# matthieugomez/LeastSquaresOptim.jl

Hardware: AMD Instinct MI355X
Metric: lm_lsmr_outer_iterations_per_sec (higher is better)
Workload: dtype f64

## Files before the change

### leastsquaresoptim.jl_amd/csrc/lsq_optimize.hip

```cpp
#include <chrono>
#include <cmath>
#include <cstring>

#include "lsq_solver.h"
#include "lsq_spmv.h"

static constexpr double MIN_DELTA = 1e-16, MAX_DELTA = 1e16, MIN_STEP_QUALITY = 1e-3;
static constexpr double MIN_DIAGONAL = 1e-6, MAX_DIAGONAL = 1e32;
static constexpr double DECREASE_THRESHOLD = 0.25, INCREASE_THRESHOLD = 0.75;

enum { SL_GRAD = 8, SL_DX = 9, SL_NONFIN = 10, SL_TRIAL = 11, SL_PRED = 12, SL_SSR = 13, SL_W0 = 14, SL_W1 = 15,
       SL_W2 = 16, SL_SUM = 17 };

extern "C" int lsq_solver_create(lsq_ctx *c, lsq_mat *J, int kind, int for_lm, lsq_solver **out) {
    LSQ_RANGE("lsq_solver_create");
    if (!c || !J || !out) return LSQ_EARG;
    if (kind == LSQ_QR && J->kind != LSQ_MAT_DENSE) {
        lsq_set_error("solver QR() is not available for sparse Jacobians. Choose between Cholesky() and LSMR()");
        return LSQ_EARG;
    }
    const bool blockdiag = kind == LSQ_CHOLESKY && J->kind == LSQ_MAT_CSC && J->bd_blocks > 0;
    const bool bordered = kind == LSQ_CHOLESKY && J->kind == LSQ_MAT_CSC && J->br_blocks > 0;
    if (kind == LSQ_CHOLESKY && J->kind != LSQ_MAT_DENSE && !blockdiag && !bordered) {
        lsq_set_error("MethodError: no AbstractAllocatedSolver for Cholesky() with a sparse Jacobian "
// ... 597 lines not shown
            (void)o->allreduce(v, 3, o->allreduce_user);
        }
        return st;
    }
};

#define CB(call)                                          \
    do {                                                  \
        if ((call) != 0) {                                \
            lsq_set_error("user callback reported failure"); \
            return LSQ_ECALLBACK;                         \
        }                                                 \
    } while (0)

static int call_g(lsq_g_callback g, lsq_mat *J, const double *x, void *user) {
    J->version++;
    if (J->kind == LSQ_MAT_CSC && !J->d_cs_user) J->csr_fresh = false;
    CB(g(J, x, user));
    return lsq_ensure_csr(J);
}
int lsq_call_g(lsq_g_callback g, lsq_mat *J, const double *x, void *user) { return call_g(g, J, x, user); }

struct IterateGuard {
    lsq_ctx *c;
    double *&x, *&fcur;
    double *x_user, *fcur_user;
    int m, n;
    ~IterateGuard() {
        if (x != x_user) lsq_d2d(c, x_user, x, (size_t)n * sizeof(double));
        if (fcur != fcur_user) lsq_d2d(c, fcur_user, fcur, (size_t)m * sizeof(double));
    }
};

static int start_residual(lsq_ctx *c, lsq_mat *J, lsq_f_callback f, void *user, double *fcur, const double *x, double *ssr,
                          int *nonfinite_at) {
    const int m = J->m, n = J->n;
    if (lsq_small_mat(J) || lsq_small_vec(m) || m <= 0) {
        CB(f(fcur, x, user));
        LSQ_TRY(lsq_sumsq(c, m, fcur, ssr));
        return lsq_first_nonfinite(c, n, x, nonfinite_at);
    }
    static_assert(SL_TRIAL == SL_NONFIN + 1, "the two scalars of the loop head travel together");
    LSQ_TRY(lsq_first_nonfinite_to_slot(c, n, x, c->d_slots + SL_NONFIN));
    LSQ_TRY(f_then_sumsq(c, false, f, user, m, fcur, x, 7, c->d_slots + SL_TRIAL));
    double sl[2];
    LSQ_TRY(lsq_read_slots(c, SL_NONFIN, 2, sl));
    *nonfinite_at = (int)sl[0];
    *ssr = sl[1];
    return LSQ_OK;
}

static int optimize_lm_loop(lsq_ctx *c, lsq_solver *sv, LoopBuffers &b, lsq_mat *J, double *x_user, double *fcur_user,
                            lsq_f_callback f, lsq_g_callback g, void *user, const lsq_options *o, lsq_result *r);
static int optimize_lm(lsq_ctx *c, lsq_solver *sv, LoopBuffers &b, lsq_mat *J, double *x_user, double *fcur_user,
                       lsq_f_callback f, lsq_g_callback g, void *user, const lsq_options *o, lsq_result *r) {
    ShardedExit ex{c, o};
    return ex.finish(optimize_lm_loop(c, sv, b, J, x_user, fcur_user, f, g, user, o, r));
}
static int optimize_lm_loop(lsq_ctx *c, lsq_solver *sv, LoopBuffers &b, lsq_mat *J, double *x_user, double *fcur_user,
                            lsq_f_callback f, lsq_g_callback g, void *user, const lsq_options *o, lsq_result *r) {
    const int m = J->m, n = J->n;
    double *x = x_user, *fcur = fcur_user, *xt = b.xt, *ftrial = b.ftrial;
    IterateGuard guard{c, x, fcur, x_user, fcur_user, m, n};
    double delta = o->delta > 0 ? o->delta : 10.0;
    double decrease_factor = 2.0;
    int f_calls = 0, g_calls = 0, mul_calls = 0, xc = 0, fc = 0, gc = 0;
    bool converged = false;
    double ssr;
    int iter = 0, nonfinite_at = -1;
    const bool sharded = o->row_allreduce != nullptr;
    if (sharded) CB(f(fcur, x, user));
    else LSQ_TRY(start_residual(c, J, f, user, fcur, x, &ssr, &nonfinite_at));
    f_calls++;
    auto rows_sum = [&](double *d_buf, int count) -> int {
        if (o->row_allreduce(d_buf, count, (void *)c->stream, o->row_allreduce_user) != 0) {
            lsq_set_error("row all-reduce callback reported failure");
            return LSQ_ECALLBACK;
        }
        return LSQ_OK;
    };
    if (sharded) {
        LSQ_TRY(sumsq_to_slot(c, false, m, fcur, 7, c->d_slots + SL_TRIAL));
        LSQ_TRY(rows_sum(c->d_slots + SL_TRIAL, 1));
        LSQ_TRY(lsq_read_slots(c, SL_TRIAL, 1, &ssr));
        LSQ_TRY(lsq_first_nonfinite(c, n, x, &nonfinite_at));
    }
    r->ssr0 = ssr;
    double maxabs_gr = INFINITY;
    bool need_jac = true;
    const int gn = ngrid(c, n);
    const bool exact = lsq_small_mat(J) && !sharded && !(sv->kind == LSQ_LSMR && sv->gen_ldiv);
    int last_inner = 0;
    const bool no_spec_grad = getenv("LSQ_NO_SPEC_GRADIENT") != nullptr;
    bool spec_launched = false, spec_grad_ready = false, spec_pending = false;
    struct SpecGuard { lsq_mat *J; bool &ready; bool &pending; ~SpecGuard() { if (ready || pending) lsq_sparse_colsum_forget(J); } }
        spec_guard{J, spec_grad_ready, spec_pending};
    int local_done = 0;
    double gssr = ssr, ggr = maxabs_gr;
    long long inner_total = 0;
    while (iter < o->iterations) {
        if (!o->allreduce && converged) break;
        if (o->allreduce && converged) {
            int all = 1;
            gssr = ssr; ggr = maxabs_gr;
            LSQ_TRY(global_exchange(o, &gssr, &ggr, &all));
            if (all) break;
            ++iter; local_done = 1;
            continue;
        }
        iter++;
        if (nonfinite_at >= 0) {
            r->bad_index = nonfinite_at;
            r->iterations = iter - 1;
            lsq_set_error("IsFiniteException: non-finite x at index %d", nonfinite_at);
            return LSQ_ENONFINITE;
        }
        if (need_jac) {
            LSQ_TRY(call_g(g, J, x, user));
            g_calls++;
            need_jac = false;
        }
        bool have_grad = false;
        if (spec_grad_ready) {
            lsq_sparse_grad_colsum_adopt(J);
            have_grad = true;
            spec_grad_ready = false;
        }
        const bool spec_ok = !no_spec_grad && !exact && !sharded && sv->kind == LSQ_LSMR && f == model_f && g == model_g &&
                             iter < o->iterations && !lsq_dbg_serial;
        spec_launched = false;
        if (!exact && J->colsum_version != J->version && lsq_can_fuse_grad_colsum(J)) {
            LSQ_TRY(lsq_sparse_grad_colsum(J, fcur, b.grad));
            have_grad = true;
        }
        const double *cs = nullptr;
        LSQ_TRY(lsq_rowshard_colsum(sv, J, &cs));
        const bool one_wg = !exact && n <= LSQ_ONE_WG_N;
        const bool lm_prep = one_wg && sv->kind == LSQ_LSMR && ssr >= 0.0 && lsq_lsmr_takes_lm_prep(sv, J);
        if (exact) LSQ_TRY(lsq_exact_lm_damp(c, n, cs, 1.0 / delta, b.dtd));
        else if (!one_wg) LSQ_LAUNCH(k_lm_damp, dim3(1), dim3(1024), 0, c->stream, n, cs, 1.0 / delta, b.dtd);
        {
            if (!have_grad) LSQ_TRY(gradient_into(c, exact, J, fcur, b.grad));
            if (sharded) LSQ_TRY(rows_sum(b.grad, n));
            if (lm_prep) {}
            else if (one_wg)
                LSQ_LAUNCH(k_lm_damp_grad, dim3(1), dim3(1024), 0, c->stream, n, cs, 1.0 / delta, b.dtd, b.grad,
                                   x, b.lo, b.hi, c->d_slots + SL_GRAD);
            else
                LSQ_LAUNCH(k_gradnorm, dim3(gn), dim3(LSQ_NT), 0, c->stream, n, b.grad, x, b.lo, b.hi,
                                   c->d_partials, lsq_ctr(c, 4), c->d_slots + SL_GRAD);
            mul_calls++;
        }
        struct Xchg { const lsq_options *o; double *gssr, *ggr; } xchg{o, &gssr, &ggr};
        if (o->allreduce) {
            gssr = ssr; ggr = maxabs_gr;
            c->idle_hook = [](void *p) -> int {
                Xchg *q = (Xchg *)p;
                int all = 0;
                return global_exchange(q->o, q->gssr, q->ggr, &all);
            };
            c->idle_user = &xchg;
            c->idle_status = 0;
            if (sv->kind != LSQ_LSMR || exact) lsq_run_idle_hook(c);
        }
        int lmiter = 0;
        struct TailCtx {
// ... 108 lines not shown
            decrease_factor *= 2.0;
        }
        record(o, c, iter, n, ssr, maxabs_gr, delta, rho, lmiter, accepted ? 1 : 0, x);
    }
    (void)local_done;
    LSQ_HIP(hipStreamSynchronize(c->stream));
    r->optimizer = LSQ_LEVENBERG_MARQUARDT;
    r->ssr = o->allreduce ? gssr : ssr;
    r->iterations = iter;
    r->converged = converged; r->x_converged = xc; r->f_converged = fc; r->g_converged = gc;
    r->f_calls = f_calls; r->g_calls = g_calls; r->mul_calls = mul_calls;
    r->lsmr_iterations = inner_total;
    return LSQ_OK;
}

static int optimize_dogleg_loop(lsq_ctx *c, lsq_solver *sv, LoopBuffers &b, lsq_mat *J, double *x, double *fcur,
                                lsq_f_callback f, lsq_g_callback g, void *user, const lsq_options *o, lsq_result *r);
static int optimize_dogleg(lsq_ctx *c, lsq_solver *sv, LoopBuffers &b, lsq_mat *J, double *x, double *fcur,
                           lsq_f_callback f, lsq_g_callback g, void *user, const lsq_options *o, lsq_result *r) {
    ShardedExit ex{c, o};
    return ex.finish(optimize_dogleg_loop(c, sv, b, J, x, fcur, f, g, user, o, r));
}
static int optimize_dogleg_loop(lsq_ctx *c, lsq_solver *sv, LoopBuffers &b, lsq_mat *J, double *x_user, double *fcur_user,
                                lsq_f_callback f, lsq_g_callback g, void *user, const lsq_options *o, lsq_result *r) {
    const int m = J->m, n = J->n;
    double *x = x_user, *fcur = fcur_user, *xt = b.xt, *ftrial = b.ftrial;
    IterateGuard guard{c, x, fcur, x_user, fcur_user, m, n};
    double delta = o->delta > 0 ? o->delta : 1.0;
    bool reuse = false, converged = false;
    double wnorm_dgn = 0.0, wnorm_dgr = 0.0, alpha = 0.0, wdot_gr_gn = 0.0;
    int f_calls = 0, g_calls = 0, mul_calls = 0, xc = 0, fc = 0, gc = 0;
    double ssr;
    int iter = 0, nonfinite_at = -1;
    LSQ_TRY(start_residual(c, J, f, user, fcur, x, &ssr, &nonfinite_at));
    f_calls++;
    r->ssr0 = ssr;
    double maxabs_gr = INFINITY;
    const int gn = ngrid(c, n);
    const bool exact = lsq_small_mat(J);
    double gssr = ssr, ggr = maxabs_gr;
    long long inner_total = 0;
    while (iter < o->iterations) {
        if (!o->allreduce && converged) break;
        if (o->allreduce && converged) {
            int all = 1;
            gssr = ssr; ggr = maxabs_gr;
            LSQ_TRY(global_exchange(o, &gssr, &ggr, &all));
            if (all) break;
            ++iter;
            continue;
        }
        iter++;
        if (nonfinite_at >= 0) {
            r->bad_index = nonfinite_at;
            r->iterations = iter - 1;
            lsq_set_error("IsFiniteException: non-finite x at index %d", nonfinite_at);
            return LSQ_ENONFINITE;
        }
        int ls_iter = 0;
        bool exchanged = false;
        if (!reuse) {
            LSQ_TRY(call_g(g, J, x, user));
            g_calls++;
            bool have_grad = false;
            if (!exact && J->colsum_version != J->version && lsq_can_fuse_grad_colsum(J)) {
                LSQ_TRY(lsq_sparse_grad_colsum(J, fcur, b.dgr));
                have_grad = true;
            }
            const double *cs = lsq_cached_colsum(J);
            if (!cs) return LSQ_EHIP;
            LSQ_LAUNCH(k_dl_scale, dim3(gn), dim3(LSQ_NT), 0, c->stream, n, cs, b.dtd);
            if (iter == 1) {
                double wx2;
                LSQ_TRY(lsq_wdot(c, n, x, x, b.dtd, &wx2));
                double wx = std::sqrt(wx2);
                if (wx > 0) delta *= wx;
            }
            if (!have_grad) LSQ_TRY(gradient_into(c, exact, J, fcur, b.dgr));
            mul_calls++;
            LSQ_LAUNCH(k_gradnorm, dim3(gn), dim3(LSQ_NT), 0, c->stream, n, b.dgr, x, b.lo, b.hi,
                               c->d_partials, lsq_ctr(c, 4), c->d_slots + SL_GRAD);
            LSQ_TRY(lsq_ediv(c, n, b.dgr, b.dtd, b.dgr));
            LSQ_TRY(wdot_to_slot(c, exact, n, b.dgr, b.dgr, b.dtd, 5, c->d_slots + SL_W0));
            LSQ_TRY(predicted_to_slot(c, exact, J, b.dgr, nullptr, b.fpred, 6, c->d_slots + SL_SUM));
            mul_calls++;
            LSQ_TRY(lsq_fill(c, n, 0.0, b.dgn));
            if (o->allreduce) {
                int all = 0;
                gssr = ssr; ggr = maxabs_gr;
                LSQ_TRY(global_exchange(o, &gssr, &ggr, &all));
                exchanged = true;
            }
            if (sv->kind == LSQ_LSMR) LSQ_TRY(lsq_lsmr_solve(sv, J, fcur, nullptr, b.dgn, &ls_iter));
            else LSQ_TRY(lsq_ldiv(sv, J, fcur, b.dgn, &ls_iter));
            mul_calls += ls_iter;
            inner_total += ls_iter / 2;
            LSQ_TRY(wdot_to_slot(c, exact, n, b.dgn, b.dgn, b.dtd, 5, c->d_slots + SL_W1));
            LSQ_TRY(wdot_to_slot(c, exact, n, b.dgr, b.dgn, b.dtd, 5, c->d_slots + SL_W2));
            LSQ_HIP(hipGetLastError());
            double sl10[10];
// ... 92 lines not shown
        LSQ_TRY(lsq_d2h(c, hx.data(), x, (size_t)n * sizeof(double)));
        int st = check_start(hx.data(), n, opt);
        if (st != LSQ_OK) {
            lsq_set_error("ArgumentError: Initial guess must be within bounds.");
            res->status = st;
            return st;
        }
    }
    LsqWorkspace *w = (LsqWorkspace *)c->workspace;
    const bool lm = optimizer == LSQ_LEVENBERG_MARQUARDT;
    if (!(w && w->J == J && w->m == J->m && w->n == J->n && w->optimizer == optimizer && w->solver_kind == solver_kind &&
          w->has_lo == (opt->h_lower != nullptr) && w->has_hi == (opt->h_upper != nullptr))) {
        lsq_workspace_free(w);
        c->workspace = nullptr;
        w = new LsqWorkspace();
        int st0 = lsq_solver_create(c, J, solver_kind, lm, &w->solver);
        if (st0 != LSQ_OK) {
            delete w;
            res->status = st0;
            return st0;
        }
        w->buf = new LoopBuffers();
        st0 = alloc_loop(*w->buf, c, J->m, J->n, opt, !lm);
        if (st0 != LSQ_OK) {
            lsq_workspace_free(w);
            res->status = st0;
            return st0;
        }
        w->J = J; w->m = J->m; w->n = J->n; w->optimizer = optimizer; w->solver_kind = solver_kind;
        w->has_lo = opt->h_lower != nullptr; w->has_hi = opt->h_upper != nullptr;
        c->workspace = w;
    } else {
        const size_t nb = (size_t)(J->n > 0 ? J->n : 1) * sizeof(double);
        LSQ_HIP(hipMemsetAsync(w->buf->dx, 0, nb, c->stream));
        if (opt->h_lower) LSQ_HIP(hipMemcpyAsync(w->buf->lo, opt->h_lower, nb, hipMemcpyHostToDevice, c->stream));
        if (opt->h_upper) LSQ_HIP(hipMemcpyAsync(w->buf->hi, opt->h_upper, nb, hipMemcpyHostToDevice, c->stream));
        if (opt->h_lower || opt->h_upper) LSQ_HIP(hipStreamSynchronize(c->stream));
    }
    if (w->solver->kind == LSQ_LSMR) {
        w->solver->precond_cb = opt->preconditioner;
        w->solver->precond_user = opt->preconditioner_user;
        w->solver->gen_update = opt->precond_update;
        w->solver->gen_ldiv = opt->precond_ldiv;
        w->solver->gen_user = opt->precond_general_user;
    }
    if (opt->row_allreduce) {
        if (!lm || w->solver->kind != LSQ_LSMR || opt->allreduce || J->kind == LSQ_MAT_OP) {
            lsq_set_error("row-sharded runs (lsq_options.row_allreduce): LevenbergMarquardt(LSMR()) on stored Jacobians only, and "
                          "not together with the independent-problems exchange (lsq_options.allreduce)");
            res->status = LSQ_EARG;
            return LSQ_EARG;
        }
        LSQ_TRY(lsq_solver_set_row_allreduce(w->solver, opt->row_allreduce, opt->row_allreduce_user,
                                             opt->global_rows > 0 ? opt->global_rows : (long long)J->m));
    } else if (w->solver->kind == LSQ_LSMR) {
        LSQ_TRY(lsq_solver_set_row_allreduce(w->solver, nullptr, nullptr, 0));
    }
    auto t0 = std::chrono::steady_clock::now();
    int st = lm ? optimize_lm(c, w->solver, *w->buf, J, x, fcur, f, g, user, opt, res)
                : optimize_dogleg(c, w->solver, *w->buf, J, x, fcur, f, g, user, opt, res);
    hipStreamSynchronize(c->stream);
    res->seconds = std::chrono::duration<double>(std::chrono::steady_clock::now() - t0).count();
    res->status = st;
    return st;
}

struct lsq_model {
    lsq_ctx *ctx;
    lsq_mat *J;
    bool fused = false;
    double *d_Acsc = nullptr;
    double *d_Acsr = nullptr;
    double *d_Ab = nullptr;
    double *d_b = nullptr;
    double *d_t = nullptr;
    double *d_s = nullptr;
    double *d_sspec = nullptr;
    const double *tanh_x = nullptr;
    const double *sfac_x = nullptr;
    double *d_b_perm = nullptr;
    double *d_perm[2] = {nullptr, nullptr};
    const double *perm_of[2] = {nullptr, nullptr};
};
static void model_perm_invalidate(lsq_model *md, const double *vec) {
    for (int k = 0; k < 2; ++k)
        if (!vec || md->perm_of[k] == vec) md->perm_of[k] = nullptr;
}

__global__ void __launch_bounds__(LSQ_NT) k_tanh(int n, const double *__restrict__ x, double *__restrict__ t) {
    for (int i = blockIdx.x * LSQ_NT + threadIdx.x; i < n; i += gridDim.x * LSQ_NT) t[i] = tanh(x[i]);
}

struct EpiResidual {
    static constexpr bool REDUCE = false;
    const int *done;
    int extra_blocks;
    const double *b;
    double *out;
    double *partials;
    unsigned *counter;
    __device__ void seg(int i, double dot, double &) const { out[i] = dot - b[i]; }
    using has_pre = void;
    __device__ double pre(int i) const { return b[i]; }
    __device__ void seg_pre(int i, double dot, double bi, double &) const { out[i] = dot - bi; }
    __device__ void extra(int, double &) const {}
    __device__ void finalize(double) const {}
};

struct EpiResidualSq {
    static constexpr bool REDUCE = true;
    const int *done;
    int extra_blocks;
    const double *b;
    double *out;
    double *partials;
    unsigned *counter;
    double *slot;
    LsqSlotPublish pub;
    __device__ void seg(int i, double dot, double &racc) const { seg_pre(i, dot, b[i], racc); }
    using has_pre = void;
    __device__ double pre(int i) const { return b[i]; }
    __device__ void seg_pre(int i, double dot, double bi, double &racc) const {
        const double v = dot - bi;
        out[i] = v;
        racc += v * v;
    }
    __device__ void extra(int, double &) const {}
    __device__ void finalize(double t) const {
        *slot = t;
        if (pub.count > 0) {
            for (int i = 0; i < pub.count; ++i)
                __hip_atomic_store(pub.dst + i, pub.src + i == slot ? t : pub.src[i], __ATOMIC_RELAXED, __HIP_MEMORY_SCOPE_SYSTEM);
            __hip_atomic_store(pub.seq_word, pub.seq, __ATOMIC_RELEASE, __HIP_MEMORY_SCOPE_SYSTEM);
        }
    }
};

__global__ void __launch_bounds__(LSQ_NT)
k_scale_cols(int n, const int *__restrict__ colptr, int m_dense, const double *__restrict__ A,
             const double *__restrict__ x, double *__restrict__ out) {
    for (int j = blockIdx.x; j < n; j += gridDim.x) {
        double t = tanh(x[j]);
        double s = 1.0 - t * t;
        long long k0 = colptr ? colptr[j] : (long long)j * m_dense;
        long long k1 = colptr ? colptr[j + 1] : (long long)(j + 1) * m_dense;
        for (long long k = k0 + threadIdx.x; k < k1; k += LSQ_NT) out[k] = A[k] * s;
    }
}
__global__ void __launch_bounds__(LSQ_NT)
k_scale_dense(int m, const double *__restrict__ A, const double *__restrict__ x, double *__restrict__ out) {
    const int j = blockIdx.x;
    const double t = tanh(x[j]);
    const double sfac = 1.0 - t * t;
    const size_t base = (size_t)j * m;
    for (int i = blockIdx.y * LSQ_NT + threadIdx.x; i < m; i += gridDim.y * LSQ_NT) out[base + i] = A[base + i] * sfac;
}
__global__ void __launch_bounds__(LSQ_NT)
k_scale_csr(long long nnz, const int *__restrict__ colidx, const double *__restrict__ A, const double *__restrict__ sfac,
            double *__restrict__ out) {
    for (long long k = blockIdx.x * (long long)LSQ_NT + threadIdx.x; k < nnz; k += (long long)gridDim.x * LSQ_NT)
        out[k] = A[k] * sfac[colidx[k]];
}
__global__ void __launch_bounds__(LSQ_NT) k_tanh_sfac(int n, const double *__restrict__ x, double *__restrict__ t,
                                                      double *__restrict__ s) {
    for (int i = blockIdx.x * LSQ_NT + threadIdx.x; i < n; i += gridDim.x * LSQ_NT) {
        const double v = tanh(x[i]);
        t[i] = v;
        s[i] = 1.0 - v * v;
    }
}
__global__ void __launch_bounds__(LSQ_NT) k_sfac(int n, const double *__restrict__ x, double *__restrict__ s) {
    for (int i = blockIdx.x * LSQ_NT + threadIdx.x; i < n; i += gridDim.x * LSQ_NT) {
        double t = tanh(x[i]);
        s[i] = 1.0 - t * t;
    }
}

__global__ void __launch_bounds__(LSQ_NT)
k_scale_bcsc(int nseg, int n, const int *__restrict__ ptr, const double *__restrict__ A, const double *__restrict__ sfac,
             double *__restrict__ out) {
    const int lane = threadIdx.x & 63, per = LSQ_NT / 64;
    for (int s = blockIdx.x * per + (threadIdx.x >> 6); s < nseg; s += gridDim.x * per) {
        const double f = sfac[s % n];
        const int k1 = ptr[s + 1];
        for (int k = ptr[s] + lane; k < k1; k += 64) out[k] = A[k] * f;
    }
}

typedef double lsq_d2 __attribute__((ext_vector_type(2)));
template <bool NT>
__global__ void __launch_bounds__(1024)
k_scale_lds(long long nnz4, const unsigned short *__restrict__ col16, const double *__restrict__ A,
            const double *__restrict__ sfac, int n, double *__restrict__ out) {
    extern __shared__ double sf[];
    for (int i = threadIdx.x; i < n; i += 1024) sf[i] = sfac[i];
    __syncthreads();
    for (long long q = blockIdx.x * 1024LL + threadIdx.x; q < nnz4; q += (long long)gridDim.x * 1024) {
        const long long k = 4 * q;
        const lsq_d2 a0 = *reinterpret_cast<const lsq_d2 *>(A + k);
        const lsq_d2 a1 = *reinterpret_cast<const lsq_d2 *>(A + k + 2);
        const uint2 c = *reinterpret_cast<const uint2 *>(col16 + k);
        lsq_d2 o0, o1;
// ... 47 lines not shown
    return hipGetLastError() == hipSuccess ? 0 : 1;
}

static void model_trial_buffers(void *user, const double *xt, double **t_out, double **s_out) {
    lsq_model *md = (lsq_model *)user;
    md->tanh_x = md->sfac_x = nullptr;
    if ((md->J->kind == LSQ_MAT_CSC && md->J->srows.active) || md->J->kind == LSQ_MAT_DENSE) {
        *t_out = md->d_t;
        *s_out = md->d_sspec;
        md->tanh_x = md->sfac_x = xt;
    }
}

static int model_f_sumsq(void *user, double *out, const double *x, int ctr, double *d_out, LsqSlotPublish pub, bool *done,
                         const int *skip) {
    lsq_model *md = (lsq_model *)user;
    lsq_ctx *c = md->ctx;
    lsq_mat *J = md->J;
    *done = false;
    if (!(J->kind == LSQ_MAT_CSC && J->srows.active)) return model_f(out, x, user);
    model_perm_invalidate(md, out);
    EpiResidualSq e{skip, 0, md->d_b, out, c->d_partials, lsq_ctr(c, ctr), d_out, pub};
    const bool have_tanh = md->tanh_x == x;
    md->tanh_x = nullptr;
    if (!have_tanh) {
        md->sfac_x = nullptr;
        LSQ_LAUNCH(k_tanh, dim3(ngrid(c, J->n)), dim3(LSQ_NT), 0, c->stream, J->n, x, md->d_t);
    }
    if (launch_sell_rows(J, nullptr, md->d_t, e, md->fused ? nullptr : md->d_Acsr) != LSQ_OK) return 1;
    *done = true;
    return hipGetLastError() == hipSuccess ? 0 : 1;
}

static int model_pair_tail(void *user, lsq_mat *J, const double *dx, const double *fcur, double *ftrial, const double *xt,
                           double *slot_pred, double *slot_trial, LsqSlotPublish pub, const int *skip, bool *done, SpecGrad *sg) {
    lsq_model *md = (lsq_model *)user;
    lsq_ctx *c = md->ctx;
    *done = false;
    if (!(md->fused && J == md->J && J->kind == LSQ_MAT_CSC && J->srows.active && J->srows.ncw == 1 && J->d_colscale &&
          J->n <= LSQ_PAIR_X_MAX && md->tanh_x == xt) || getenv("LSQ_NO_PAIR_TAIL"))
        return 0;
    const LsqSell &S = J->srows;
    const int nxpad = (J->n + 1) & ~1;
    const size_t lds = (size_t)std::max(2 * nxpad, LSQ_SELL_ROWS_MAX) * sizeof(double);
    if (lsq_set_lds(c, (const void *)k_sell_rows_pair<0>, (size_t)2 * LSQ_PAIR_X_MAX * sizeof(double)) != LSQ_OK) return 0;
    const size_t plen = (size_t)S.nslices * 64;
    const int pgrid = std::max(1, std::min(lsq_div_up((long long)plen, LSQ_NT), c->num_cus * 8));
    if (!md->d_b_perm) {
        double *pb = nullptr, *p0 = nullptr, *p1 = nullptr;
        if (hipMalloc(&pb, plen * sizeof(double)) != hipSuccess || hipMalloc(&p0, plen * sizeof(double)) != hipSuccess ||
            hipMalloc(&p1, plen * sizeof(double)) != hipSuccess) {
            (void)hipGetLastError();
            hipFree(pb); hipFree(p0); hipFree(p1);
            return 0;
        }
        md->d_b_perm = pb; md->d_perm[0] = p0; md->d_perm[1] = p1;
        LSQ_LAUNCH(k_sell_perm_rows<0>, dim3(pgrid), dim3(LSQ_NT), 0, c->stream, sell_dev(S), S.wrows, S.nslices, (const double *)md->d_b,
                   md->d_b_perm);
    }
    int k = md->perm_of[0] == fcur ? 0 : (md->perm_of[1] == fcur ? 1 : -1);
    if (k < 0) {
        k = 0;
        LSQ_LAUNCH(k_sell_perm_rows<0>, dim3(pgrid), dim3(LSQ_NT), 0, c->stream, sell_dev(S), S.wrows, S.nslices, fcur, md->d_perm[k]);
        md->perm_of[k] = fcur;
    }
    md->perm_of[1 - k] = ftrial;
    md->tanh_x = nullptr;
    const int grid = std::max(1, std::min(S.nblocks, c->num_cus));
    const bool spec = sg && sg->gate && md->sfac_x == xt;
    SellPairEpi e{skip, md->d_perm[k], md->d_b_perm, ftrial, md->d_perm[1 - k], c->d_partials, c->d_partials + 4096, lsq_ctr(c, 7),
                  slot_pred, slot_trial, pub, spec ? sg->gate : nullptr, spec ? sg->ssr : 0.0, MIN_STEP_QUALITY,
                  c->d_slots + SL_SSR};
    LSQ_LAUNCH(k_sell_rows_pair<0>, dim3(grid), dim3(LSQ_BIG_NT), lds, c->stream, sell_dev(S), S.wrows, J->m, dx, J->d_colscale,
               (const double *)md->d_t, J->n, nxpad, e);
    *done = true;
    if (hipGetLastError() != hipSuccess) return 1;
    if (spec) {
        const int st = lsq_sparse_grad_colsum_spec(J, ftrial, sg->grad, md->d_sspec, sg->gate);
        if (st == LSQ_OK) sg->launched = true;
        else if (st != LSQ_EARG) return 1;
    }
    return 0;
}

static int model_g(lsq_mat *J, const double *x, void *user) {
    lsq_model *md = (lsq_model *)user;
    lsq_ctx *c = md->ctx;
    if (J->kind == LSQ_MAT_DENSE) {}
    else if (md->sfac_x == x) std::swap(md->d_s, md->d_sspec);
    else LSQ_LAUNCH(k_sfac, dim3(ngrid(c, J->n)), dim3(LSQ_NT), 0, c->stream, J->n, x, md->d_s);
    md->sfac_x = nullptr;
    md->tanh_x = nullptr;
// ... 55 lines not shown
        }
        J->csr_fresh = true;
    } else {
        const long long tot = (long long)J->m * J->n;
        const int chunks = std::max(1, (int)std::min<long long>((J->m + 4 * LSQ_NT - 1) / (4 * LSQ_NT),
                                                               std::max<long long>(1, (long long)c->num_cus * 16 / std::max(1, J->n))));
        if (tot > 0)
            LSQ_LAUNCH(k_scale_dense, dim3(J->n, chunks), dim3(LSQ_NT), 0, c->stream, J->m, md->d_Acsc, x, J->d_dense);
    }
    J->version++;
    return hipGetLastError() == hipSuccess ? 0 : 1;
}

extern "C" lsq_f_callback lsq_model_f(void) { return model_f; }
extern "C" lsq_g_callback lsq_model_g(void) { return model_g; }

extern "C" int lsq_model_tanh_create(lsq_ctx *c, lsq_mat *J, const double *hA, const double *hb, lsq_model **out) {
    if (!c || !J || !hA || !hb || !out) return LSQ_EARG;
    LSQ_HIP(hipSetDevice(c->device));
    lsq_model *md = new lsq_model();
    md->ctx = c;
    md->J = J;
    const size_t nb = (size_t)(J->n > 0 ? J->n : 1) * sizeof(double);
    LSQ_HIP(hipMalloc(&md->d_b, (size_t)(J->m > 0 ? J->m : 1) * sizeof(double)));
    LSQ_HIP(hipMemcpy(md->d_b, hb, (size_t)J->m * sizeof(double), hipMemcpyHostToDevice));
    LSQ_HIP(hipMalloc(&md->d_t, nb));
    LSQ_HIP(hipMalloc(&md->d_s, nb));
    LSQ_HIP(hipMalloc(&md->d_sspec, nb));
    if (lsq_colscale_fusable(J)) {
        LSQ_TRY(lsq_mat_set_values(J, hA));
        LSQ_TRY(lsq_fill(c, J->n, 1.0, md->d_s));
        LSQ_TRY(lsq_mat_set_colscale(J, md->d_s));
        md->fused = true;
        LSQ_HIP(hipStreamSynchronize(c->stream));
        *out = md;
        return LSQ_OK;
    }
    size_t vb = (size_t)(J->nnz + 8) * sizeof(double);
    LSQ_HIP(hipMalloc(&md->d_Acsc, vb));
    LSQ_ZERO(md->d_Acsc, 0, vb);
    LSQ_HIP(hipMemcpy(md->d_Acsc, hA, (size_t)J->nnz * sizeof(double), hipMemcpyHostToDevice));
    if (J->kind == LSQ_MAT_CSC) {
        const size_t rb = (size_t)(lsq_mirror_rows_len(J) + 1024) * sizeof(double);
        LSQ_HIP(hipMalloc(&md->d_Acsr, rb));
        LSQ_ZERO(md->d_Acsr, 0, rb);
        LSQ_TRY(lsq_mirror_rows(J, md->d_Acsc, md->d_Acsr));
        if (lsq_mirror_cols_len(J) > 0) {
            const size_t cbytes = (size_t)(lsq_mirror_cols_len(J) + 1024) * sizeof(double);
            LSQ_HIP(hipMalloc(&md->d_Ab, cbytes));
            LSQ_ZERO(md->d_Ab, 0, cbytes);
            LSQ_TRY(lsq_mirror_cols(J, md->d_Acsc, md->d_Ab));
        }
        LSQ_HIP(hipStreamSynchronize(c->stream));
    }
    *out = md;
    return LSQ_OK;
}

extern "C" int lsq_model_destroy(lsq_model *md) {
    if (!md) return LSQ_OK;
    hipStreamSynchronize(md->ctx->stream);
    if (md->fused && md->J) lsq_mat_set_colscale(md->J, nullptr);
    hipFree(md->d_Acsc); hipFree(md->d_Acsr); hipFree(md->d_Ab); hipFree(md->d_b); hipFree(md->d_t); hipFree(md->d_s); hipFree(md->d_sspec);
    hipFree(md->d_b_perm); hipFree(md->d_perm[0]); hipFree(md->d_perm[1]);
    delete md;
    return LSQ_OK;
// ... 2 lines not shown
```

### leastsquaresoptim.jl_amd/csrc/lsq_sell.h

```cpp
#pragma once

constexpr int LSQ_SELL_POS_BITS = 13;
constexpr unsigned LSQ_SELL_POS_MASK = (1u << LSQ_SELL_POS_BITS) - 1u;
constexpr int LSQ_SELL_ROWS_MAX = 4096;
constexpr int LSQ_SELL_CW_AUTO = 6;
constexpr int LSQ_SELL_CW_MAX = 32;
constexpr int LSQ_SELL_GROWS_MAX = 16384;
constexpr int LSQ_SELL_CCOLS_MAX = 2560;

struct SellDev {
    const int2 *smeta;
    const unsigned *info;
    const unsigned short *idx16;
    const double *val;
    int nblocks;
    int spw;
};

template <int U>
struct SellBatch {
    double2 a[U];
    unsigned c[U];
};
template <int U, bool CLAMP>
// ... 88 lines not shown
    sell_lane_sum_from<SQ>(vp, ip, 0, L, len, xl, sum, sq, lane);
}

struct SellSliceRef {
    int2 sm;
    unsigned inf;
};
__device__ __forceinline__ SellSliceRef sell_slice_ref(const SellDev &S, int s, int s1, int lane) {
    SellSliceRef r;
    r.sm = make_int2(0, 0);
    r.inf = LSQ_SELL_POS_MASK;
    if (s < s1) {
        r.sm = S.smeta[__builtin_amdgcn_readfirstlane(s)];
        r.inf = S.info[(size_t)s * 64 + lane];
    }
    return r;
}
template <bool SQ, class Out>
__device__ __forceinline__ void sell_wave_slices(const SellDev &S, int s0, int s1, int wv, int lane, const double *xl, Out out) {
    constexpr int NW = LSQ_BIG_NT / 64;
    int s = s0 + wv;
    SellSliceRef A = sell_slice_ref(S, s, s1, lane);
    __syncthreads();
    for (; s < s1; s += NW) {
        const SellSliceRef a = A;
        A = sell_slice_ref(S, s + NW, s1, lane);
        const size_t oa = (size_t)a.sm.x + lane * 2;
        const unsigned pos = a.inf & LSQ_SELL_POS_MASK;
        double sum = 0.0, sq = 0.0;
        sell_lane_sum<SQ>(S.val + oa, S.idx16 + oa, a.sm.y, (int)(a.inf >> LSQ_SELL_POS_BITS), xl, sum, sq, lane);
        if (pos != LSQ_SELL_POS_MASK) out(pos, sum, sq);
    }
}

template <class Epi>
__global__ void __launch_bounds__(LSQ_BIG_NT) k_sell_rows(SellDev S, int wrows, int m, const double *__restrict__ x,
                                                          const double *__restrict__ xscale, int nx, int nxpad, Epi epi) {
    extern __shared__ __attribute__((aligned(16))) double smem[];
    __shared__ double sh[LSQ_BIG_NT / 64];
    double *xl = smem;
    double *yw = smem + nxpad;
    const int tid = threadIdx.x, lane = tid & 63, wv = tid >> 6;
    constexpr int XR = (LSQ_LDS_X_MAX + LSQ_BIG_NT - 1) / LSQ_BIG_NT;
    double xr[XR];
#pragma unroll
    for (int q = 0; q < XR; ++q) xr[q] = x[min(tid + q * LSQ_BIG_NT, nx - 1)];
    if (xscale) {
        double sr[XR];
#pragma unroll
        for (int q = 0; q < XR; ++q) sr[q] = xscale[min(tid + q * LSQ_BIG_NT, nx - 1)];
#pragma unroll
        for (int q = 0; q < XR; ++q) xr[q] *= sr[q];
    }
    const int dflag = epi.done ? *epi.done : 0;

    if constexpr (EpiHasBlockPrepare<Epi>::value) epi.block_prepare();
    if constexpr (EpiHasPrepare<Epi>::value) epi.prepare();
#pragma unroll
    for (int q = 0; q < XR; ++q)
        if (tid + q * LSQ_BIG_NT < nx) xl[tid + q * LSQ_BIG_NT] = xr[q];
    if (dflag) return;
    constexpr int Q = LSQ_SELL_ROWS_MAX / LSQ_BIG_NT;
    double racc = 0.0;
    for (int w = blockIdx.x; w < S.nblocks; w += gridDim.x) {
        const int base = w * wrows, rows = min(wrows, m - base);
        const int s0 = w * S.spw, s1 = s0 + S.spw;
        double pre[Q];
        if constexpr (EpiHasPre<Epi>::value) {
#pragma unroll
            for (int q = 0; q < Q; ++q) pre[q] = epi.pre(base + min(tid + q * LSQ_BIG_NT, rows - 1));
        }
        sell_wave_slices<false>(S, s0, s1, wv, lane, xl, [&](unsigned pos, double sum, double) { yw[pos] = sum; });
        __syncthreads();
#pragma unroll
        for (int q = 0; q < Q; ++q) {
            const int i = tid + q * LSQ_BIG_NT;
            if (i < rows) {
                if constexpr (EpiHasPre<Epi>::value) epi.seg_pre(base + i, yw[i], pre[q], racc);
                else epi.seg(base + i, yw[i], racc);
            }
        }
    }
    for (int e = blockIdx.x; e < epi.extra_blocks; e += gridDim.x)
        if (tid < LSQ_NT) epi.extra(e, racc);
    finish_block_nt<LSQ_BIG_NT>(epi, racc, sh);
}

template <int U, bool CLAMP>
__device__ __forceinline__ void sell_batch_sum2(SellBatch<U> &B, int p0, int np, int len, const double *xa, const double *xb,
                                                double &sa, double &sb) {
#pragma unroll
    for (int u = 0; u < U; ++u) {
        const unsigned i0 = B.c[u] & 0xffffu, i1 = B.c[u] >> 16;
        double a0 = B.a[u].x * xa[i0], a1 = B.a[u].y * xa[i1], b0 = B.a[u].x * xb[i0], b1 = B.a[u].y * xb[i1];
        asm volatile("" : "+v"(a0), "+v"(a1), "+v"(b0), "+v"(b1));
        const int j = 2 * (p0 + u);
        const bool pin = !CLAMP || p0 + u < np;
        const bool in0 = pin && j < len, in1 = pin && j + 1 < len;
        const double ta0 = sa + a0;
        sa = in0 ? ta0 : sa;
        const double ta1 = sa + a1;
        sa = in1 ? ta1 : sa;
        const double tb0 = sb + b0;
        sb = in0 ? tb0 : sb;
        const double tb1 = sb + b1;
// ... 326 lines not shown
```

### leastsquaresoptim.jl_amd/csrc/lsq_spmv.h

```cpp
#pragma once
#include <hip/hip_ext.h>

#include <algorithm>
#include <type_traits>
#include <utility>

#include "lsq_common.h"

constexpr int LSQ_TILE_WINDOW = 2048;
constexpr int LSQ_TILE_NNZ = LSQ_TILE_WINDOW - 3;
constexpr int LSQ_TILE_SEGS = LSQ_NT;

struct SegsDev {
    const int *ptr;
    const int *idx;
    const double *val;
    const int *tiles;
    const unsigned short *idx16;
    const int *order;
    int nseg;
    int ntiles;
    int nnz;
};

// ... 138 lines not shown

constexpr int LSQ_BIG_NT = 1024;
constexpr int LSQ_BIG_WINDOW = 8 * LSQ_BIG_NT;
constexpr int LSQ_BIG_NNZ = LSQ_BIG_WINDOW - 3;
constexpr int LSQ_BIG_SEGS = LSQ_BIG_NT;
constexpr int LSQ_LDS_X_MAX = 12160;

template <bool IDX16>
__device__ __forceinline__ int4 load_idx4(const SegsDev &S, int k) {
    if constexpr (IDX16) {
        const uint2 p = *reinterpret_cast<const uint2 *>(S.idx16 + k);
        return make_int4((int)(p.x & 0xffffu), (int)(p.x >> 16), (int)(p.y & 0xffffu), (int)(p.y >> 16));
    } else {
        return *reinterpret_cast<const int4 *>(S.idx + k);
    }
}

struct BigTileRegs {
    double2 v0[2], v1[2];
    int4 ci[2];
    int4 meta;
    int pa, pe;
    double pre;
};

template <class E, class = void>
struct EpiHasPrepare : std::false_type {};
template <class E>
struct EpiHasPrepare<E, std::void_t<typename E::has_prepare>> : std::true_type {};
template <class E, class = void>
struct EpiHasPre : std::false_type {};
template <class E>
struct EpiHasPre<E, std::void_t<typename E::has_pre>> : std::true_type {};

template <class Epi, bool IDX16>
__global__ void __launch_bounds__(LSQ_BIG_NT) k_seg_stream_lds(SegsDev S, const int4 *__restrict__ meta, int nbig,
                                                               const double *__restrict__ x, int nx, int nxpad,
                                                               Epi epi) {
    extern __shared__ __attribute__((aligned(16))) double smem[];
    __shared__ double sh[LSQ_BIG_NT / 64];
    double *xl = smem;
    double *prod = smem + nxpad;
    const int tid = threadIdx.x;
    const int G = gridDim.x;
    constexpr bool HAS_PRE = EpiHasPre<Epi>::value;
    const int kmax = (S.nnz + 3) & ~3;
    auto load_meta = [&](int tb) {
        int4 mt = meta[tb < nbig ? tb : nbig - 1];
        if (tb >= nbig) mt.y = mt.x;
        return mt;
    };
    auto load_data = [&](BigTileRegs &r, int4 mt) {
        r.meta = mt;
        const int ka = mt.z & ~3;
#pragma unroll
        for (int c = 0; c < 2; ++c) {
            const int k = min(ka + c * 4 * LSQ_BIG_NT + 4 * tid, kmax);
            r.v0[c] = *reinterpret_cast<const double2 *>(S.val + k);
            r.v1[c] = *reinterpret_cast<const double2 *>(S.val + k + 2);
            r.ci[c] = load_idx4<IDX16>(S, k);
        }
        const int s = min(mt.x + tid, S.nseg - 1);
        r.pa = S.ptr[s];
        r.pe = S.ptr[s + 1];
        if constexpr (HAS_PRE) r.pre = epi.pre(s);
    };
// ... 675 lines not shown
```

Baseline: 3987.

## Fuse model start residual with nonfinite check and defer the start readback

```diff
diff --git a/leastsquaresoptim.jl_amd/csrc/lsq_optimize.hip b/leastsquaresoptim.jl_amd/csrc/lsq_optimize.hip
--- a/leastsquaresoptim.jl_amd/csrc/lsq_optimize.hip
+++ b/leastsquaresoptim.jl_amd/csrc/lsq_optimize.hip
@@ -653,15 +653,39 @@
     }
 };
 
-static int start_residual(lsq_ctx *c, lsq_mat *J, lsq_f_callback f, void *user, double *fcur, const double *x, double *ssr,
-                          int *nonfinite_at) {
+static bool model_start_applies(lsq_f_callback f, lsq_g_callback g, void *user, lsq_mat *J, const lsq_options *o);
+static int model_start(void *user, double *fcur, const double *x, double *dx, double *slot_nonfin, double *slot_ssr,
+                       LsqSlotPublish pub);
+static int start_finish(lsq_ctx *c, LsqSlotPublish *pending, double *ssr, int *nonfinite_at) {
+    double sl[2];
+    const unsigned long long seq = pending->seq;
+    pending->count = 0;
+    LSQ_TRY(lsq_wait_slots(c, SL_NONFIN, 2, seq, sl));
+    *nonfinite_at = (int)sl[0];
+    *ssr = sl[1];
+    return LSQ_OK;
+}
+static int start_residual(lsq_ctx *c, lsq_mat *J, lsq_f_callback f, lsq_g_callback g, void *user, const lsq_options *o,
+                          double *fcur, const double *x, double *dx, double *ssr, int *nonfinite_at, LsqSlotPublish *defer) {
     const int m = J->m, n = J->n;
+    static_assert(SL_TRIAL == SL_NONFIN + 1, "the two scalars of the loop head travel together");
+    if (model_start_applies(f, g, user, J, o)) {
+        LsqSlotPublish pub = lsq_slots_ticket(c, SL_NONFIN, 2);
+        if (model_start(user, fcur, x, dx, c->d_slots + SL_NONFIN, c->d_slots + SL_TRIAL, pub) != 0) {
+            lsq_set_error("user callback reported failure");
+            return LSQ_ECALLBACK;
+        }
+        if (defer && o->iterations > 0 && !lsq_dbg_serial) {
+            *defer = pub;
+            return LSQ_OK;
+        }
+        return start_finish(c, &pub, ssr, nonfinite_at);
+    }
     if (lsq_small_mat(J) || lsq_small_vec(m) || m <= 0) {
         CB(f(fcur, x, user));
         LSQ_TRY(lsq_sumsq(c, m, fcur, ssr));
         return lsq_first_nonfinite(c, n, x, nonfinite_at);
     }
-    static_assert(SL_TRIAL == SL_NONFIN + 1, "the two scalars of the loop head travel together");
     LSQ_TRY(lsq_first_nonfinite_to_slot(c, n, x, c->d_slots + SL_NONFIN));
     LSQ_TRY(f_then_sumsq(c, false, f, user, m, fcur, x, 7, c->d_slots + SL_TRIAL));
     double sl[2];
@@ -690,8 +714,12 @@
     double ssr;
     int iter = 0, nonfinite_at = -1;
     const bool sharded = o->row_allreduce != nullptr;
+    LsqSlotPublish start_pub;
+    struct StartGuard { lsq_mat *J; LsqSlotPublish &p; ~StartGuard() { if (p.count > 0) lsq_sparse_colsum_forget(J); } }
+        start_guard{J, start_pub};
+    ssr = 0.0;
     if (sharded) CB(f(fcur, x, user));
-    else LSQ_TRY(start_residual(c, J, f, user, fcur, x, &ssr, &nonfinite_at));
+    else LSQ_TRY(start_residual(c, J, f, g, user, o, fcur, x, b.dx, &ssr, &nonfinite_at, &start_pub));
     f_calls++;
     auto rows_sum = [&](double *d_buf, int count) -> int {
         if (o->row_allreduce(d_buf, count, (void *)c->stream, o->row_allreduce_user) != 0) {
@@ -753,6 +781,18 @@
         if (!exact && J->colsum_version != J->version && lsq_can_fuse_grad_colsum(J)) {
             LSQ_TRY(lsq_sparse_grad_colsum(J, fcur, b.grad));
             have_grad = true;
+        }
+        if (start_pub.count > 0) {
+            LsqSlotPublish p = start_pub;
+            LSQ_TRY(start_finish(c, &p, &ssr, &nonfinite_at));
+            r->ssr0 = gssr = ssr;
+            if (nonfinite_at >= 0) {
+                r->bad_index = nonfinite_at;
+                r->iterations = 0;
+                lsq_set_error("IsFiniteException: non-finite x at index %d", nonfinite_at);
+                return LSQ_ENONFINITE;
+            }
+            start_pub.count = 0;
         }
         const double *cs = nullptr;
         LSQ_TRY(lsq_rowshard_colsum(sv, J, &cs));
@@ -927,7 +967,11 @@
     int f_calls = 0, g_calls = 0, mul_calls = 0, xc = 0, fc = 0, gc = 0;
     double ssr;
     int iter = 0, nonfinite_at = -1;
-    LSQ_TRY(start_residual(c, J, f, user, fcur, x, &ssr, &nonfinite_at));
+    LsqSlotPublish start_pub;
+    struct StartGuard { lsq_mat *J; LsqSlotPublish &p; ~StartGuard() { if (p.count > 0) lsq_sparse_colsum_forget(J); } }
+        start_guard{J, start_pub};
+    ssr = 0.0;
+    LSQ_TRY(start_residual(c, J, f, g, user, o, fcur, x, b.dx, &ssr, &nonfinite_at, &start_pub));
     f_calls++;
     r->ssr0 = ssr;
     double maxabs_gr = INFINITY;
@@ -961,6 +1005,18 @@
             if (!exact && J->colsum_version != J->version && lsq_can_fuse_grad_colsum(J)) {
                 LSQ_TRY(lsq_sparse_grad_colsum(J, fcur, b.dgr));
                 have_grad = true;
+            }
+            if (start_pub.count > 0) {
+                LsqSlotPublish p = start_pub;
+                LSQ_TRY(start_finish(c, &p, &ssr, &nonfinite_at));
+                r->ssr0 = gssr = ssr;
+                if (nonfinite_at >= 0) {
+                    r->bad_index = nonfinite_at;
+                    r->iterations = 0;
+                    lsq_set_error("IsFiniteException: non-finite x at index %d", nonfinite_at);
+                    return LSQ_ENONFINITE;
+                }
+                start_pub.count = 0;
             }
             const double *cs = lsq_cached_colsum(J);
             if (!cs) return LSQ_EHIP;
@@ -1119,7 +1175,7 @@
         c->workspace = w;
     } else {
         const size_t nb = (size_t)(J->n > 0 ? J->n : 1) * sizeof(double);
-        LSQ_HIP(hipMemsetAsync(w->buf->dx, 0, nb, c->stream));
+        if (!model_start_applies(f, g, user, J, opt)) LSQ_HIP(hipMemsetAsync(w->buf->dx, 0, nb, c->stream));
         if (opt->h_lower) LSQ_HIP(hipMemcpyAsync(w->buf->lo, opt->h_lower, nb, hipMemcpyHostToDevice, c->stream));
         if (opt->h_upper) LSQ_HIP(hipMemcpyAsync(w->buf->hi, opt->h_upper, nb, hipMemcpyHostToDevice, c->stream));
         if (opt->h_lower || opt->h_upper) LSQ_HIP(hipStreamSynchronize(c->stream));
@@ -1173,6 +1229,31 @@
     for (int k = 0; k < 2; ++k)
         if (!vec || md->perm_of[k] == vec) md->perm_of[k] = nullptr;
 }
+static bool model_sliced_fused(const lsq_model *md) {
+    const lsq_mat *J = md->J;
+    return md->fused && J && J->kind == LSQ_MAT_CSC && J->srows.active && J->srows.ncw == 1 && J->d_colscale;
+}
+static bool model_pair_ready(const lsq_model *md) {
+    return model_sliced_fused(md) && md->J->n <= LSQ_PAIR_X_MAX && md->d_b_perm && !getenv("LSQ_NO_PAIR_TAIL");
+}
+static void model_build_mirrors(lsq_model *md) {
+    if (!(model_sliced_fused(md) && md->J->n <= LSQ_PAIR_X_MAX) || md->d_b_perm) return;
+    lsq_ctx *c = md->ctx;
+    const LsqSell &S = md->J->srows;
+    const size_t plen = (size_t)S.nslices * 64;
+    double *pb = nullptr, *p0 = nullptr, *p1 = nullptr;
+    if (hipMalloc(&pb, plen * sizeof(double)) != hipSuccess || hipMalloc(&p0, plen * sizeof(double)) != hipSuccess ||
+        hipMalloc(&p1, plen * sizeof(double)) != hipSuccess) {
+        (void)hipGetLastError();
+        hipFree(pb); hipFree(p0); hipFree(p1);
+        return;
+    }
+    md->d_b_perm = pb; md->d_perm[0] = p0; md->d_perm[1] = p1;
+    model_perm_invalidate(md, nullptr);
+    const int pgrid = std::max(1, std::min(lsq_div_up((long long)plen, LSQ_NT), c->num_cus * 8));
+    LSQ_LAUNCH(k_sell_perm_rows<0>, dim3(pgrid), dim3(LSQ_NT), 0, c->stream, sell_dev(S), S.wrows, S.nslices, (const double *)md->d_b,
+               md->d_b_perm);
+}
 
 __global__ void __launch_bounds__(LSQ_NT) k_tanh(int n, const double *__restrict__ x, double *__restrict__ t) {
     for (int i = blockIdx.x * LSQ_NT + threadIdx.x; i < n; i += gridDim.x * LSQ_NT) t[i] = tanh(x[i]);
@@ -1223,6 +1304,14 @@
     }
 };
 
+struct EpiResidualSqMirror : EpiResidualSq {
+    using has_slice_mirror = void;
+    const double *b_perm;
+    double *out_perm;
+    __device__ double slice_pre(size_t k) const { return b_perm[k]; }
+    __device__ void slice_out(size_t k, double dot, double bk) const { out_perm[k] = dot - bk; }
+};
+
 __global__ void __launch_bounds__(LSQ_NT)
 k_scale_cols(int n, const int *__restrict__ colptr, int m_dense, const double *__restrict__ A,
              const double *__restrict__ x, double *__restrict__ out) {
@@ -1248,13 +1337,23 @@
     for (long long k = blockIdx.x * (long long)LSQ_NT + threadIdx.x; k < nnz; k += (long long)gridDim.x * LSQ_NT)
         out[k] = A[k] * sfac[colidx[k]];
 }
-__global__ void __launch_bounds__(LSQ_NT) k_tanh_sfac(int n, const double *__restrict__ x, double *__restrict__ t,
-                                                      double *__restrict__ s) {
+__global__ void __launch_bounds__(LSQ_NT)
+k_model_start(int n, const double *__restrict__ x, double *__restrict__ t, double *__restrict__ s, double *__restrict__ dx,
+              double *partials, unsigned *counter, double *out_nonfin) {
+    __shared__ double sh[LSQ_NT / 64];
+    double code = 0.0;
     for (int i = blockIdx.x * LSQ_NT + threadIdx.x; i < n; i += gridDim.x * LSQ_NT) {
-        const double v = tanh(x[i]);
+        const double xi = x[i];
+        const double v = tanh(xi);
         t[i] = v;
         s[i] = 1.0 - v * v;
-    }
+        dx[i] = 0.0;
+        if (!isfinite(xi) && code == 0.0) code = 1e15 - (double)(i + 1);
+    }
+    const double bv = block_max<LSQ_NT>(code, sh);
+    grid_reduce<LSQ_NT, true>(bv, partials, counter, gridDim.x, sh, [=](double m) {
+        *out_nonfin = (m == 0.0) ? -1.0 : (1e15 - m) - 1.0;
+    });
 }
 __global__ void __launch_bounds__(LSQ_NT) k_sfac(int n, const double *__restrict__ x, double *__restrict__ s) {
     for (int i = blockIdx.x * LSQ_NT + threadIdx.x; i < n; i += gridDim.x * LSQ_NT) {
@@ -1368,32 +1467,43 @@
     return hipGetLastError() == hipSuccess ? 0 : 1;
 }
 
+static bool model_start_applies(lsq_f_callback f, lsq_g_callback g, void *user, lsq_mat *J, const lsq_options *o) {
+    if (f != model_f || g != model_g || !user || o->row_allreduce) return false;
+    const lsq_model *md = (const lsq_model *)user;
+    return J == md->J && model_sliced_fused(md) && J->n > 0 && !(lsq_small_mat(J) || lsq_small_vec(J->m));
+}
+static int model_start(void *user, double *fcur, const double *x, double *dx, double *slot_nonfin, double *slot_ssr,
+                       LsqSlotPublish pub) {
+    lsq_model *md = (lsq_model *)user;
+    lsq_ctx *c = md->ctx;
+    lsq_mat *J = md->J;
+    LSQ_LAUNCH(k_model_start, dim3(ngrid(c, J->n)), dim3(LSQ_NT), 0, c->stream, J->n, x, md->d_t, md->d_sspec, dx, c->d_partials,
+               lsq_ctr(c, 0), slot_nonfin);
+    md->tanh_x = nullptr;
+    md->sfac_x = x;
+    model_perm_invalidate(md, fcur);
+    EpiResidualSq e{nullptr, 0, md->d_b, fcur, c->d_partials, lsq_ctr(c, 7), slot_ssr, pub};
+    if (model_pair_ready(md)) {
+        EpiResidualSqMirror em{e, md->d_b_perm, md->d_perm[0]};
+        if (launch_sell_rows(J, nullptr, md->d_t, em) != LSQ_OK) return 1;
+        md->perm_of[0] = fcur;
+        if (md->perm_of[1] == fcur) md->perm_of[1] = nullptr;
+    } else if (launch_sell_rows(J, nullptr, md->d_t, e) != LSQ_OK) return 1;
+    return hipGetLastError() == hipSuccess ? 0 : 1;
+}
+
 static int model_pair_tail(void *user, lsq_mat *J, const double *dx, const double *fcur, double *ftrial, const double *xt,
                            double *slot_pred, double *slot_trial, LsqSlotPublish pub, const int *skip, bool *done, SpecGrad *sg) {
     lsq_model *md = (lsq_model *)user;
     lsq_ctx *c = md->ctx;
     *done = false;
-    if (!(md->fused && J == md->J && J->kind == LSQ_MAT_CSC && J->srows.active && J->srows.ncw == 1 && J->d_colscale &&
-          J->n <= LSQ_PAIR_X_MAX && md->tanh_x == xt) || getenv("LSQ_NO_PAIR_TAIL"))
-        return 0;
+    if (!(J == md->J && model_pair_ready(md) && md->tanh_x == xt)) return 0;
     const LsqSell &S = J->srows;
     const int nxpad = (J->n + 1) & ~1;
     const size_t lds = (size_t)std::max(2 * nxpad, LSQ_SELL_ROWS_MAX) * sizeof(double);
     if (lsq_set_lds(c, (const void *)k_sell_rows_pair<0>, (size_t)2 * LSQ_PAIR_X_MAX * sizeof(double)) != LSQ_OK) return 0;
     const size_t plen = (size_t)S.nslices * 64;
     const int pgrid = std::max(1, std::min(lsq_div_up((long long)plen, LSQ_NT), c->num_cus * 8));
-    if (!md->d_b_perm) {
-        double *pb = nullptr, *p0 = nullptr, *p1 = nullptr;
-        if (hipMalloc(&pb, plen * sizeof(double)) != hipSuccess || hipMalloc(&p0, plen * sizeof(double)) != hipSuccess ||
-            hipMalloc(&p1, plen * sizeof(double)) != hipSuccess) {
-            (void)hipGetLastError();
-            hipFree(pb); hipFree(p0); hipFree(p1);
-            return 0;
-        }
-        md->d_b_perm = pb; md->d_perm[0] = p0; md->d_perm[1] = p1;
-        LSQ_LAUNCH(k_sell_perm_rows<0>, dim3(pgrid), dim3(LSQ_NT), 0, c->stream, sell_dev(S), S.wrows, S.nslices, (const double *)md->d_b,
-                   md->d_b_perm);
-    }
     int k = md->perm_of[0] == fcur ? 0 : (md->perm_of[1] == fcur ? 1 : -1);
     if (k < 0) {
         k = 0;
@@ -1515,6 +1625,7 @@
         LSQ_TRY(lsq_fill(c, J->n, 1.0, md->d_s));
         LSQ_TRY(lsq_mat_set_colscale(J, md->d_s));
         md->fused = true;
+        model_build_mirrors(md);
         LSQ_HIP(hipStreamSynchronize(c->stream));
         *out = md;
         return LSQ_OK;
diff --git a/leastsquaresoptim.jl_amd/csrc/lsq_sell.h b/leastsquaresoptim.jl_amd/csrc/lsq_sell.h
--- a/leastsquaresoptim.jl_amd/csrc/lsq_sell.h
+++ b/leastsquaresoptim.jl_amd/csrc/lsq_sell.h
@@ -144,6 +144,25 @@
         if (pos != LSQ_SELL_POS_MASK) out(pos, sum, sq);
     }
 }
+template <class Pre, class Out>
+__device__ __forceinline__ void sell_wave_slices_mirror(const SellDev &S, int s0, int s1, int wv, int lane, const double *xl, Pre pre,
+                                                        Out out) {
+    constexpr int NW = LSQ_BIG_NT / 64;
+    int s = s0 + wv;
+    SellSliceRef A = sell_slice_ref(S, s, s1, lane);
+    __syncthreads();
+    for (; s < s1; s += NW) {
+        const SellSliceRef a = A;
+        A = sell_slice_ref(S, s + NW, s1, lane);
+        const size_t k = (size_t)s * 64 + lane;
+        const double p = pre(k);
+        const size_t oa = (size_t)a.sm.x + lane * 2;
+        const unsigned pos = a.inf & LSQ_SELL_POS_MASK;
+        double sum = 0.0, sq = 0.0;
+        sell_lane_sum<false>(S.val + oa, S.idx16 + oa, a.sm.y, (int)(a.inf >> LSQ_SELL_POS_BITS), xl, sum, sq, lane);
+        if (pos != LSQ_SELL_POS_MASK) out(pos, k, sum, p);
+    }
+}
 
 template <class Epi>
 __global__ void __launch_bounds__(LSQ_BIG_NT) k_sell_rows(SellDev S, int wrows, int m, const double *__restrict__ x,
@@ -182,7 +201,14 @@
 #pragma unroll
             for (int q = 0; q < Q; ++q) pre[q] = epi.pre(base + min(tid + q * LSQ_BIG_NT, rows - 1));
         }
-        sell_wave_slices<false>(S, s0, s1, wv, lane, xl, [&](unsigned pos, double sum, double) { yw[pos] = sum; });
+        if constexpr (EpiHasSliceMirror<Epi>::value)
+            sell_wave_slices_mirror(S, s0, s1, wv, lane, xl, [&](size_t k) { return epi.slice_pre(k); },
+                                    [&](unsigned pos, size_t k, double sum, double p) {
+                                        yw[pos] = sum;
+                                        epi.slice_out(k, sum, p);
+                                    });
+        else
+            sell_wave_slices<false>(S, s0, s1, wv, lane, xl, [&](unsigned pos, double sum, double) { yw[pos] = sum; });
         __syncthreads();
 #pragma unroll
         for (int q = 0; q < Q; ++q) {
diff --git a/leastsquaresoptim.jl_amd/csrc/lsq_spmv.h b/leastsquaresoptim.jl_amd/csrc/lsq_spmv.h
--- a/leastsquaresoptim.jl_amd/csrc/lsq_spmv.h
+++ b/leastsquaresoptim.jl_amd/csrc/lsq_spmv.h
@@ -194,6 +194,10 @@
 struct EpiHasPre : std::false_type {};
 template <class E>
 struct EpiHasPre<E, std::void_t<typename E::has_pre>> : std::true_type {};
+template <class E, class = void>
+struct EpiHasSliceMirror : std::false_type {};
+template <class E>
+struct EpiHasSliceMirror<E, std::void_t<typename E::has_slice_mirror>> : std::true_type {};
 
 template <class Epi, bool IDX16>
 __global__ void __launch_bounds__(LSQ_BIG_NT) k_seg_stream_lds(SegsDev S, const int4 *__restrict__ meta, int nbig,
```

After: 4065, median of 6. 2.0% higher.
